# ipc-sim/IPC

Measured on NVIDIA H100. Metric: newton_iteration_ms_assembly_ccd, lower is better.
Workload: dtype f64

## Files before the change

ipc_b200/csrc/abi.h:

```cpp
#pragma once
#include "../../include/ipcgpu.h"
#include "common.cuh"
#include "context.h"
#include <cstddef>
#include <string>

#define CK(call)                                                                                  \
    do {                                                                                          \
        cudaError_t e_ = (call);                                                                  \
        if (e_ != cudaSuccess) {                                                                  \
            ctx->err = std::string(#call) + ": " + cudaGetErrorString(e_);                        \
            return IPCGPU_ERR_CUDA;                                                               \
        }                                                                                         \
    } while (0)
#define REQUIRE(cond, code, msg)                                                                  \
    do {                                                                                          \
        if (!(cond)) {                                                                            \
            ctx->err = (msg);                                                                     \
            return (code);                                                                        \
        }                                                                                         \
    } while (0)
#define ALLOC(buf, count) REQUIRE((buf).reserve(count), IPCGPU_ERR_CUDA, "cudaMalloc failed for " #buf)

static inline int nblk(long long n, int b) { return (int)((n + b - 1) / b); }

enum Chain { kSerial, kStepBound, kDerivative };

inline int join_deriv(ipcgpu_ctx* ctx)
{
    if (!ctx->deriv_open) return IPCGPU_OK;
    ctx->deriv_open = false;
    CK(cudaEventRecord(ctx->ev_deriv_done, ctx->deriv));
    CK(cudaStreamWaitEvent(ctx->stream, ctx->ev_deriv_done, 0));
    return IPCGPU_OK;
}

inline int enter(ipcgpu_ctx* ctx, Chain chain)
{
    CK(cudaSetDevice(ctx->device));
    if (chain == kStepBound) return IPCGPU_OK;
    if (chain == kSerial || ctx->nranks > 1 || ctx->profiling) return join_deriv(ctx);
    if (ctx->deriv_open) return IPCGPU_OK;
    CK(cudaEventRecord(ctx->ev_deriv_fork, ctx->stream));
    CK(cudaStreamWaitEvent(ctx->deriv, ctx->ev_deriv_fork, 0));
    ctx->deriv_open = true;
    return IPCGPU_OK;
}
#define ENTER(chain)                                                                              \
    do {                                                                                          \
        int re_ = enter(ctx, (chain));                                                            \
        if (re_) return re_;                                                                      \
    } while (0)

int join_copy_stream(ipcgpu_ctx* ctx);
int fetch_iter_state(ipcgpu_ctx* ctx);
int sync_pattern_mirror(ipcgpu_ctx* ctx);
int flag_status(ipcgpu_ctx* ctx, unsigned mask);
void set_local(ipcgpu_ctx* ctx, unsigned bits, bool local);
int energy_result(ipcgpu_ctx* ctx, int slot, double* E, bool fetch = false, unsigned check = 0);
int energy_tail(ipcgpu_ctx* ctx, int slot, const double* partials, int n_partials, double scale, cudaEvent_t pe, double* E, bool fetch = false,
    unsigned check = 0, const double* scale_dev = nullptr);

inline bool kappa_on_device(double kappa) { return kappa == IPCGPU_KAPPA_DEVICE; }
inline const double* kappa_ptr(ipcgpu_ctx* ctx, double kappa) { return kappa_on_device(kappa) ? &ctx->iter.p->kappa : nullptr; }
#define REQUIRE_KAPPA(kappa)                                                                                                        \
    REQUIRE(!kappa_on_device(kappa) || ctx->nranks == 1, IPCGPU_ERR_STATE, "the device-resident kappa (IPCGPU_KAPPA_DEVICE) runs on one rank")
int gradient_roundtrip_begin(ipcgpu_ctx* ctx, const double* g_in);
int gradient_roundtrip_end(ipcgpu_ctx* ctx, double* g_out);
int hessian_begin(ipcgpu_ctx* ctx, Chain chain, const double* a_inout);
int hessian_end(ipcgpu_ctx* ctx, double* a_inout, unsigned check);

int nccl_sum(ipcgpu_ctx* ctx, double* buf, size_t n, const char* what);
int nccl_sum(ipcgpu_ctx* ctx, int* buf, size_t n, const char* what);
int nccl_min_u64(ipcgpu_ctx* ctx, unsigned long long* word);
int nccl_all_gather(ipcgpu_ctx* ctx, const int4* send, int4* recv, size_t n, const char* what);
void nccl_comm_destroy(ipcgpu_ctx* ctx);

int build_maps(ipcgpu_ctx* ctx);
void owned_value_range(ipcgpu_ctx* ctx);
int ensure_offsets(ipcgpu_ctx* ctx);
int upload_dir(ipcgpu_ctx* ctx, const double* p);

int timestep_prepare(ipcgpu_ctx* ctx, ipcgpu::DynamicsArgs* p);

namespace ipcgpu {
struct SortedGrid;
}
int contact_alloc(ipcgpu_ctx* ctx);
int contact_constraint_set(ipcgpu_ctx* ctx, double dHat, int wantCand, int* nC, int* nPara, int* nCand);
int contact_sync_counts(ipcgpu_ctx* ctx);
void contact_pack_lists(ipcgpu_ctx* ctx);
void contact_unpack_lists(ipcgpu_ctx* ctx);
ipcgpu::SurfArgs surf_args(const ipcgpu_ctx* ctx);
ipcgpu::BarrierArgs barrier_args(ipcgpu_ctx* ctx, double dHat, double kappa, int projectDBC);
ipcgpu::HalfSpaceArgs halfspace_args(ipcgpu_ctx* ctx);
ipcgpu::SortedGrid edge_grid(const ipcgpu_ctx* ctx);
int boxes_and_grid(ipcgpu_ctx* ctx, double radius, bool with_vertex_boxes);

int ccd_alloc(ipcgpu_ctx* ctx);
int ccd_narrow(ipcgpu_ctx* ctx, const int2* cand, const int* n32, const unsigned long long* n64, unsigned long long cap, int share, double tol, const double* err_vf,
    const double* err_ee, int stage, const int* overflow);
int ccd_build_swept(ipcgpu_ctx* ctx, double h);
int ccd_full(ipcgpu_ctx* ctx, double tol, const double* err_vf, const double* err_ee);
int ccd_read_back(ipcgpu_ctx* ctx, double* alpha_out);

int decide(ipcgpu_ctx* ctx, int op, double a, int b, cudaGraphConditionalHandle h, bool* word, const double* aux = nullptr);
int cond_prepare(ipcgpu_ctx* ctx, const char* what);

template <typename Body>
int cond_node(ipcgpu_ctx* ctx, bool loop, int op, double a, int b, Body body)
{
    int rc;
    if (!ctx->capturing) {
        bool go = false;
        if ((rc = decide(ctx, op, a, b, 0, &go))) return rc;
        while (go) {
            if ((rc = body())) return rc;
            if (!loop) break;
            if ((rc = decide(ctx, op, a, b, 0, &go))) return rc;
        }
        return IPCGPU_OK;
    }
    REQUIRE(ctx->cond_depth < ipcgpu_ctx::kCondDepth, IPCGPU_ERR_STATE, "conditional nodes nested too deeply");
    cudaStreamCaptureStatus cs;
    cudaGraph_t g = nullptr;
    const cudaGraphNode_t* deps = nullptr;
    size_t nd = 0;
    CK(cudaStreamGetCaptureInfo(ctx->stream, &cs, nullptr, &g, &deps, &nd));
    cudaGraphConditionalHandle h = 0;
    const cudaError_t eh = cudaGraphConditionalHandleCreate(&h, g, 0, 0);
    if (eh != cudaSuccess) {
        cudaGetLastError();
        ctx->err = std::string("conditional graph nodes need CUDA 12.4 or newer in the driver: ") + cudaGetErrorString(eh);
        return IPCGPU_ERR_CUDA;
    }
    if ((rc = decide(ctx, op, a, b, h, nullptr))) return rc;
    CK(cudaStreamGetCaptureInfo(ctx->stream, &cs, nullptr, &g, &deps, &nd));
    cudaGraphNodeParams np = {};
    np.type = cudaGraphNodeTypeConditional;
    np.conditional.handle = h;
    np.conditional.type = loop ? cudaGraphCondTypeWhile : cudaGraphCondTypeIf;
    np.conditional.size = 1;
    cudaGraphNode_t node;
    CK(cudaGraphAddNode(&node, g, deps, nd, &np));
    cudaGraph_t bg = np.conditional.phGraph_out[0];
    ctx->capture_bodies.push_back(bg);
    cudaStream_t outer = ctx->stream, inner = ctx->cond_streams[ctx->cond_depth];
    CK(cudaStreamBeginCaptureToGraph(inner, bg, nullptr, nullptr, 0, cudaStreamCaptureModeThreadLocal));
    ctx->stream = inner;
    ++ctx->cond_depth;
    ctx->inputs_marked = false;
    rc = body();
    if (!rc && loop) rc = decide(ctx, op, a, b, h, nullptr);
    --ctx->cond_depth;
    ctx->stream = outer;
    cudaGraph_t captured = nullptr;
    const cudaError_t ee = cudaStreamEndCapture(inner, &captured);
    if (rc) return rc;
    CK(ee);
    CK(cudaStreamUpdateCaptureDependencies(outer, &node, 1, cudaStreamSetCaptureDependencies));
    ctx->mark_inputs();
    return IPCGPU_OK;
}

constexpr int kKrylovBurst = 25;
int solver_finish(ipcgpu_ctx* ctx);
template <typename Iteration>
int krylov_loops(ipcgpu_ctx* ctx, int max_iter, Iteration iteration)
{
    for (const int burst : { kKrylovBurst, max_iter % kKrylovBurst }) {
        if (burst == 0 || burst > max_iter) continue;
        int rc = cond_node(ctx, true, ipcgpu::kSolveBurst, 0.0, burst, [&]() {
            for (int k = 0; k < burst; ++k) iteration();
            CK(cudaGetLastError());
            return IPCGPU_OK;
        });
        if (rc) return rc;
    }
    return solver_finish(ctx);
}
int solver_full_pattern(ipcgpu_ctx* ctx);
int solver_forget_full_pattern(ipcgpu_ctx* ctx);
constexpr int kPcgSpmvBlocks = ipcgpu::kSMs * 8;
int solver_pcg(ipcgpu_ctx* ctx, const double* rhs_dev, double sign, double rel_tol, int max_iter, bool multilevel);
// ... 37 lines not shown
```

ipc_b200/csrc/ccd.cu:

```cuda
#include "broadphase.cuh"
#include "abi.h"
#include <cub/cub.cuh>

namespace ipcgpu {

__global__ void __launch_bounds__(256) k_ref_ranges(SurfArgs s, const double* __restrict__ dir, const IterState* __restrict__ st, int* __restrict__ vmin, int* __restrict__ vmax)
{
    const int i = blockIdx.x * blockDim.x + threadIdx.x;
    if (i >= s.nSV) return;
    const double alpha = st->alpha_grid, inv_h = st->ref_inv_h;
    const int v = s.SVI[i];
#pragma unroll
    for (int c = 0; c < 3; ++c) {
        const double x = s.V[(size_t)c * s.nV + v];
        const double xt = x + alpha * dir[3 * (size_t)v + c];
        const int a = (int)floor((x - st->ref_lo[c]) * inv_h), b = (int)floor((xt - st->ref_lo[c]) * inv_h);
        vmin[3 * (size_t)v + c] = min(a, b);
        vmax[3 * (size_t)v + c] = max(a, b);
    }
}

__global__ void __launch_bounds__(256) k_swept_bounds(SurfArgs s, const double* __restrict__ dir, const IterState* __restrict__ st, unsigned long long* __restrict__ bounds)
{
    __shared__ double sm[6][8];
    const double alpha = st->alpha_grid;
    double r[6] = { 1e300, 1e300, 1e300, -1e300, -1e300, -1e300 };
    for (int i = blockIdx.x * blockDim.x + threadIdx.x; i < max(s.nV, s.nSV); i += gridDim.x * blockDim.x) {
        if (i < s.nV) {
#pragma unroll
            for (int c = 0; c < 3; ++c) {
                const double x = s.V[(size_t)c * s.nV + i];
                r[c] = fmin(r[c], x);
                r[3 + c] = fmax(r[3 + c], x);
            }
        }
        if (i < s.nSV) {
            const int v = s.SVI[i];
#pragma unroll
            for (int c = 0; c < 3; ++c) {
                const double xt = s.V[(size_t)c * s.nV + v] + alpha * dir[3 * (size_t)v + c];
                r[c] = fmin(r[c], xt);
                r[3 + c] = fmax(r[3 + c], xt);
            }
        }
    }
#pragma unroll
    for (int q = 0; q < 6; ++q) {
        double x = r[q];
#pragma unroll
        for (int o = 16; o > 0; o >>= 1) {
            const double y = __shfl_xor_sync(0xffffffffu, x, o);
            x = q < 3 ? fmin(x, y) : fmax(x, y);
        }
        if ((threadIdx.x & 31) == 0) sm[q][threadIdx.x >> 5] = x;
    }
    __syncthreads();
    if (threadIdx.x < 6) {
        const int q = threadIdx.x;
        double x = sm[q][0];
        for (int w = 1; w < (int)(blockDim.x >> 5); ++w) x = q < 3 ? fmin(x, sm[q][w]) : fmax(x, sm[q][w]);
        if (q < 3) atomicMin(bounds + q, flip_ord(x));
        else atomicMax(bounds + q, flip_ord(x));
    }
}

__global__ void k_swept_alpha(IterState* st, const double* __restrict__ pSize_ptr, double h, unsigned long long* __restrict__ bounds)
{
    if (threadIdx.x != 0) return;
    const double pSize = *pSize_ptr;
    double alpha = ord_to_dbl(st->step_ord);
    const double span = alpha * pSize / h;
    if (span > 1) alpha /= span;
    st->step_ord = dbl_to_ord(alpha);
    st->alpha_grid = alpha;
    st->alpha_stage[2] = alpha;
    for (int c = 0; c < 3; ++c) { bounds[c] = ~0ull; bounds[3 + c] = 0ull; }
}
__global__ void k_refgrid_params(IterState* st, const unsigned long long* __restrict__ bounds, double h, SweptCells* __restrict__ sc)
{
    if (threadIdx.x != 0) return;
    sc->lmax = 0;
    sc->hmax[0] = sc->hmax[1] = sc->hmax[2] = 0;
    double lo[3], hi[3], rmax = 0.0;
    double inv_h = 1.0 / h;
    bool bad = false;
    for (int c = 0; c < 3; ++c) {
        lo[c] = unflip_ord(bounds[c]);
        hi[c] = unflip_ord(bounds[3 + c]);
        st->ref_lo[c] = lo[c];
        st->ref_count[c] = (int)ceil((hi[c] - lo[c]) * inv_h);
        rmax = fmax(rmax, hi[c] - lo[c]);
        if (st->ref_count[c] <= 0) bad = true;
    }
    if (bad) {
        inv_h = 1.0 / (rmax * 1.01);
        st->ref_count[0] = st->ref_count[1] = st->ref_count[2] = 1;
    }
    st->ref_inv_h = inv_h;
}

constexpr int kSweptExactK = 65534;

DEV bool ranges_overlap(const int* alo, const int* ahi, const int* blo, const int* bhi)
{
    return !(blo[0] > ahi[0] || bhi[0] < alo[0] || blo[1] > ahi[1] || bhi[1] < alo[1] || blo[2] > ahi[2] || bhi[2] < alo[2]);
}
DEV void prim_range(const int* __restrict__ vmin, const int* __restrict__ vmax, const int* vs, int n, int* lo, int* hi)
{
#pragma unroll
    for (int c = 0; c < 3; ++c) {
        lo[c] = vmin[3 * (size_t)vs[0] + c];
        hi[c] = vmax[3 * (size_t)vs[0] + c];
        for (int k = 1; k < n; ++k) {
            lo[c] = min(lo[c], vmin[3 * (size_t)vs[k] + c]);
            hi[c] = max(hi[c], vmax[3 * (size_t)vs[k] + c]);
        }
    }
}
DEV bool dbc_v(const SurfArgs& s, int v) { return s.dbc && s.dbc[v] != 0; }
DEV int cod_v(const SurfArgs& s, int v) { return s.vCoDim ? s.vCoDim[v] : 3; }

DEV int swept_prim(const SurfArgs& s, int i, int* vs, int& id)
{
    if (i < s.nSF) {
        id = i;
        vs[0] = s.SF[i]; vs[1] = s.SF[(size_t)s.nSF + i]; vs[2] = s.SF[(size_t)2 * s.nSF + i];
        return 3;
    }
    i -= s.nSF;
    if (i < s.nSE) {
        id = i;
        vs[0] = s.SE[2 * i]; vs[1] = s.SE[2 * i + 1];
        return 2;
    }
    id = i - s.nSE;
    vs[0] = s.SVI[id];
    return 1;
}

__global__ void __launch_bounds__(256) k_swept_extent(SurfArgs s, const int* __restrict__ vmin, const int* __restrict__ vmax, SweptCells* __restrict__ sc)
{
    __shared__ int sm[4][8];
    int r[4] = { 0, 0, 0, 0 };
    for (int i = blockIdx.x * blockDim.x + threadIdx.x; i < s.nSF + s.nSE + s.nSV; i += gridDim.x * blockDim.x) {
        int vs[3], id, lo[3], hi[3];
        const int nv = swept_prim(s, i, vs, id);
        prim_range(vmin, vmax, vs, nv, lo, hi);
        for (int c = 0; c < 3; ++c) {
            r[0] = max(r[0], hi[c] - lo[c] + 1);
            r[1 + c] = max(r[1 + c], hi[c]);
        }
    }
    for (int q = 0; q < 4; ++q) {
        r[q] = __reduce_max_sync(0xffffffffu, r[q]);
        if ((threadIdx.x & 31) == 0) sm[q][threadIdx.x >> 5] = r[q];
    }
    __syncthreads();
    if (threadIdx.x < 4) {
        int x = 0;
        for (int w = 0; w < (int)(blockDim.x >> 5); ++w) x = max(x, sm[threadIdx.x][w]);
        atomicMax(threadIdx.x == 0 ? &sc->lmax : &sc->hmax[threadIdx.x - 1], x);
    }
}
__global__ void k_swept_cells(SweptCells* sc)
{
    if (threadIdx.x != 0) return;
    auto fits = [&](long long K) {
        unsigned long long n = 1;
        for (int c = 0; c < 3; ++c) n *= (unsigned long long)(sc->hmax[c] / K + 1);
        return n <= (unsigned long long)kGridCells;
    };
    long long lo = max(2, sc->lmax - 1);
    if (!fits(lo)) {
        long long hi = (long long)max(sc->hmax[0], max(sc->hmax[1], sc->hmax[2])) + 1;
        while (hi - lo > 1) {
            const long long mid = (lo + hi) / 2;
            if (fits(mid)) hi = mid;
            else lo = mid;
        }
        lo = hi;
    }
    const int K = (int)min(lo, 0x7fffffffll);
    sc->K = K;
    for (int c = 0; c < 3; ++c) sc->n[c] = sc->hmax[c] / K + 1;
}
DEV unsigned swept_key(const SweptCells& g, int type, int x, int y, int z) { return ((unsigned)type << kGridCellsLog2) | (unsigned)((z * g.n[1] + y) * g.n[0] + x); }

__global__ void __launch_bounds__(256) k_swept_count(SurfArgs s, const int* __restrict__ vmin, const int* __restrict__ vmax, const SweptCells* __restrict__ sc,
    int* __restrict__ cnt)
{
    const int i = blockIdx.x * blockDim.x + threadIdx.x;
    if (i >= s.nSF + s.nSE + s.nSV) return;
    const SweptCells g = *sc;
    int vs[3], id, lo[3], hi[3];
    const int nv = swept_prim(s, i, vs, id);
    prim_range(vmin, vmax, vs, nv, lo, hi);
    for (int z = lo[2] / g.K; z <= hi[2] / g.K; ++z)
        for (int y = lo[1] / g.K; y <= hi[1] / g.K; ++y)
            for (int x = lo[0] / g.K; x <= hi[0] / g.K; ++x) atomicAdd(cnt + swept_key(g, 3 - nv, x, y, z), 1);
}
__global__ void __launch_bounds__(256) k_swept_scatter(SurfArgs s, const int* __restrict__ vmin, const int* __restrict__ vmax, const SweptCells* __restrict__ sc,
    int* __restrict__ cnt, const int* __restrict__ off, unsigned* __restrict__ keys, uint4* __restrict__ ent)
{
    const int i = blockIdx.x * blockDim.x + threadIdx.x;
    if (i >= s.nSF + s.nSE + s.nSV) return;
    const SweptCells g = *sc;
    int vs[3], id, lo[3], hi[3];
    const int nv = swept_prim(s, i, vs, id);
    prim_range(vmin, vmax, vs, nv, lo, hi);
    auto rel = [&](int v, int c) { return (unsigned)min(max((long long)v - ((long long)g.K * c - 1), 0ll), 65535ll); };
    for (int z = lo[2] / g.K; z <= hi[2] / g.K; ++z)
        for (int y = lo[1] / g.K; y <= hi[1] / g.K; ++y)
            for (int x = lo[0] / g.K; x <= hi[0] / g.K; ++x) {
                const unsigned key = swept_key(g, 3 - nv, x, y, z);
                const int pos = off[key] + atomicSub(cnt + key, 1) - 1;
                keys[pos] = key;
                ent[pos] = make_uint4(rel(lo[0], x) | (rel(lo[1], y) << 16), rel(lo[2], z) | (rel(hi[0], x) << 16), rel(hi[1], y) | (rel(hi[2], z) << 16), (unsigned)id);
            }
}

DEV bool swept_hit(const uint4& a, const uint4& b)
{
    const unsigned M01 = __vmaxu2(a.x, b.x), m01 = __vminu2(__funnelshift_r(a.y, a.z, 16), __funnelshift_r(b.y, b.z, 16));
    const unsigned M2 = max(a.y & 0xffffu, b.y & 0xffffu), m2 = min(a.z >> 16, b.z >> 16);
    return __vcmpleu2(M01, m01) == 0xffffffffu && (M01 & 0xffffu) != 0u && (M01 >> 16) != 0u && M2 != 0u && M2 <= m2;
}

struct CandOut {
    int2* cand;
    unsigned long long* n;
    unsigned long long cap;
    int* overflow;
};
DEV void push_cand(const CandOut& o, int2 c)
{
    const unsigned m = __activemask();
    const int lane = threadIdx.x & 31, leader = __ffs(m) - 1;
    unsigned long long base = 0;
    if (lane == leader) base = atomicAdd(o.n, (unsigned long long)__popc(m));
    base = __shfl_sync(m, base, leader);
    const unsigned long long i = base + __popc(m & ((1u << lane) - 1u));
    if (i < o.cap) o.cand[i] = c;
    else atomicExch(o.overflow, 1);
}

struct SweptArgs {
    SurfArgs s;
    const double* dir;
    const IterState* st;
    const int *vmin, *vmax;
    const SweptCells* sc;
    const unsigned* keys;
    const uint4* ent;
    const int* off;
    int lo, hi;
    CandOut out;
};

DEV void pt_candidate(const SweptArgs& a, bool wide, int svI, int sfI)
{
    const SurfArgs& s = a.s;
    const int vI = s.SVI[svI];
    const int tv[3] = { s.SF[sfI], s.SF[(size_t)s.nSF + sfI], s.SF[(size_t)2 * s.nSF + sfI] };
    if (wide) {
        int lo[3], hi[3];
        prim_range(a.vmin, a.vmax, tv, 3, lo, hi);
        if (!ranges_overlap(a.vmin + 3 * (size_t)vI, a.vmax + 3 * (size_t)vI, lo, hi)) return;
    }
    const bool oP = obstacle_vertex(s, vI), oT = obstacle_vertex(s, tv[0]);
    if (oP && oT) return;
    if (!oP && !oT && ((cod_v(s, vI) < 3 && cod_v(s, tv[0]) < 3) || (dbc_v(s, vI) && dbc_v(s, tv[0]) && dbc_v(s, tv[1]) && dbc_v(s, tv[2])))) return;
    push_cand(a.out, make_int2(-svI - 1, sfI));
}
DEV void ee_candidate(const SweptArgs& a, bool wide, int eI, int eJ)
{
    const SurfArgs& s = a.s;
    if (eI < a.lo || eI >= a.hi) return;
    const int v[4] = { s.SE[2 * eI], s.SE[2 * eI + 1], s.SE[2 * eJ], s.SE[2 * eJ + 1] };
    if (wide) {
        int qlo[3], qhi[3], lo[3], hi[3];
        prim_range(a.vmin, a.vmax, v, 2, qlo, qhi);
        prim_range(a.vmin, a.vmax, v + 2, 2, lo, hi);
        if (!ranges_overlap(qlo, qhi, lo, hi)) return;
    }
    {
        const double alpha = a.st->alpha_grid;
        double blo[2][3], bhi[2][3];
#pragma unroll
        for (int e = 0; e < 2; ++e)
#pragma unroll
            for (int c = 0; c < 3; ++c) {
                blo[e][c] = 1e300;
                bhi[e][c] = -1e300;
#pragma unroll
                for (int k = 0; k < 2; ++k) {
                    const int w = v[2 * e + k];
                    const double x = __ldg(s.V + (size_t)c * s.nV + w), xt = x + alpha * __ldg(a.dir + 3 * (size_t)w + c);
                    blo[e][c] = fmin(fmin(blo[e][c], x), xt);
                    bhi[e][c] = fmax(fmax(bhi[e][c], x), xt);
                }
            }
// ... 1083 lines not shown
                            ms_in = 0.0; tolerance_in = a.tol; t_max = max_t0; iter = 0; is_impacting = false; best = nullptr;
                            restart = true;
                        }
                        else {
                            if (attempt == 1 && hit) toi *= 0.8;
                            finished = true;
                        }
                    }
                }
                if (restart) {
                    width_tolerances(vf, P, tolerance_in, tol);
#pragma unroll
                    for (int d = 0; d < 3; ++d) inv_tol[d] = 1.0 / tol[d];
                    bfs1_init(bf, bufA, bufB, tolerance_in, best);
                    out_tol = tolerance_in;
                }
                if (finished) {
                    if (hit == 1) atomicMin(min_ord, dbl_to_ord(toi));
                    busy = false;
                }
            }
        }
    }
}

__global__ void __launch_bounds__(128, 2) k_ti_stage2(NarrowArgs a, const unsigned* __restrict__ survivors, const unsigned* __restrict__ nSurvPtr, unsigned* __restrict__ work,
    DBox* __restrict__ scratch, int cap, unsigned long long* __restrict__ min_ord, int* __restrict__ warn)
{
    __shared__ DBox sLevels[kStage2WarpsPerCtaDev][2][kSmemLevel];
    __shared__ TiPair sPair[kStage2WarpsPerCtaDev];
    const int lane = threadIdx.x & 31;
    const int warp_global = (blockIdx.x * blockDim.x + threadIdx.x) >> 5;
    DBox* sA = sLevels[threadIdx.x >> 5][0];
    DBox* sB = sLevels[threadIdx.x >> 5][1];
    DBox* bufA = scratch + (size_t)warp_global * 2 * cap;
    DBox* bufB = bufA + cap;
    const unsigned nSurv = *nSurvPtr;
    unsigned long long boxes = 0;
    for (;;) {
        unsigned w = 0;
        if (lane == 0) w = atomicAdd(work, 1u);
        w = __shfl_sync(0xffffffffu, w, 0);
        if (w >= nSurv) {
            if (lane == 0 && boxes) atomicAdd(reinterpret_cast<unsigned long long*>(warn + 7), boxes);
            break;
        }
        bool vf;
        {
            int v[4];
            TiPair Pl;
            load_pair(a.s, a.dir, a.cand[survivors[w]], vf, v, Pl);
            if (lane == 0) sPair[threadIdx.x >> 5] = Pl;
            __syncwarp();
        }
        const TiPair& P = sPair[threadIdx.x >> 5];
        double toi;
        const long long t0 = clock64();
        const int hit = pair_ccd(vf, P, a, bufA, bufB, cap, lane, toi, warn, boxes, sA, sB);
        if (hit && lane == 0) atomicMin(min_ord, dbl_to_ord(toi));
        if (lane == 0) {
            const unsigned dt = (unsigned)((clock64() - t0) >> 6);
            atomicMax(reinterpret_cast<unsigned*>(warn + 3), dt);
            atomicAdd(reinterpret_cast<unsigned*>(warn + 4), dt);
        }
        __syncwarp();
    }
}

__global__ void k_ccd_init(IterState* st, const int* __restrict__ n32, const unsigned long long* __restrict__ n64, unsigned long long cap, int rank, int nranks, int share,
    double seed, unsigned* nSurv, unsigned* work, int* flags)
{
    if (threadIdx.x != 0) return;
    const double alpha = ord_to_dbl(st->step_ord);
    st->max_t = alpha;
    st->ccd_ord = (seed >= 0.0 && seed < alpha) ? dbl_to_ord(seed) : st->step_ord;
    unsigned long long n = n32 ? (unsigned long long)max(*n32, 0) : *n64;
    if (n > cap) n = cap;
    st->cand_range[0] = share ? n * rank / nranks : 0ull;
    st->cand_range[1] = share ? n * (rank + 1) / nranks : n;
    *nSurv = 0;
    *work = 0;
    for (int q = 0; q < 12; ++q) flags[q] = 0;
}
__global__ void k_ccd_finish(IterState* st, const unsigned* __restrict__ nSurv, const int* __restrict__ flags, const int* __restrict__ overflow, int is_full)
{
    if (threadIdx.x != 0) return;
    if (flags[0]) {
        st->ccd_ord = 0ull;
        st->flags[FLAG_ZERO_CCD_DISTANCE] = 1;
    }
    if (overflow && *overflow) st->flags[FLAG_CCD_CAPACITY] = 1;
    st->flags[FLAG_TI_WARNINGS] += flags[1];
    st->ccd_stats[0] = *nSurv;
    st->ccd_stats[1] = (unsigned long long)flags[1];
    st->ccd_stats[2] = (unsigned)flags[2];
    st->ccd_stats[3] = (unsigned long long)(unsigned)flags[4] << 6;
    st->ccd_stats[4] = (unsigned long long)(unsigned)flags[5] << 6;
    st->ccd_stats[5] = *reinterpret_cast<const unsigned long long*>(flags + 6);
    st->ccd_stats[6] = *reinterpret_cast<const unsigned long long*>(flags + 8);
    st->ccd_stats[7] = st->cand_range[1] - st->cand_range[0];
    if (is_full) st->n_full_cand = st->ccd_stats[7];
}
__global__ void k_ccd_commit(IterState* st, int stage)
{
    if (threadIdx.x != 0) return;
    st->step_ord = st->ccd_ord;
    st->alpha_stage[stage] = ord_to_dbl(st->ccd_ord);
}

}

using namespace ipcgpu;


constexpr int kStage2WarpsPerCta = 4;
constexpr int kStage2Ctas = kSMs * 2;
constexpr int kLevelCap = 4096;

int ccd_alloc(ipcgpu_ctx* ctx)
{
    CcdWork& w = ctx->ccd;
    const size_t warps = (size_t)kStage2Ctas * kStage2WarpsPerCta;
    const size_t nEnt = (size_t)8 * std::max(ctx->nSF + ctx->nSE + ctx->nSV, 1);
    size_t scan_bytes = 0;
    cub::DeviceScan::ExclusiveSum(nullptr, scan_bytes, (int*)nullptr, (int*)nullptr, (int)(3 * kGridCells + 1));
    if (!w.arena_lock.p) {
        if (!w.arena_lock.reserve(1) || cudaMemsetAsync(w.arena_lock.p, 0, sizeof(int), ctx->stream) != cudaSuccess) {
            ctx->err = "CCD workspace allocation failed";
            return IPCGPU_ERR_CUDA;
        }
    }
    bool ok = w.arena.reserve((size_t)2 * kArenaLevel * sizeof(DBox)) && w.vmin.reserve((size_t)3 * ctx->nV) && w.vmax.reserve((size_t)3 * ctx->nV) && w.cand.reserve(ctx->ccd_capacity) && w.surv.reserve(ctx->ccd_capacity) && w.surv2.reserve(ctx->ccd_capacity)
        && w.scratch.reserve(warps * 2 * kLevelCap * sizeof(DBox)) && w.counters.reserve(16) && w.ncand.reserve(2) && w.bounds.reserve(8) && w.cells.reserve(1)
        && w.sw_keys.reserve(nEnt) && w.sw_ent.reserve(nEnt) && w.sw_cnt.reserve((size_t)3 * kGridCells + 1) && w.sw_off.reserve((size_t)3 * kGridCells + 1)
        && w.sw_tmp.reserve(scan_bytes + 256);
    if (!ok) {
        ctx->err = "CCD workspace allocation failed";
        return IPCGPU_ERR_CUDA;
    }
    return 0;
}

int ccd_narrow(ipcgpu_ctx* ctx, const int2* cand, const int* n32, const unsigned long long* n64, unsigned long long cap, int share, double tol, const double* err_vf,
    const double* err_ee, int stage, const int* overflow)
{
    CcdWork& w = ctx->ccd;
    cudaStream_t st = ctx->stream;
    NarrowArgs a;
    a.s = surf_args(ctx);
    a.dir = ctx->dir.p;
    a.cand = cand;
    for (int c = 0; c < 3; ++c) { a.err_vf[c] = err_vf[c]; a.err_ee[c] = err_ee[c]; }
    a.tol = tol;
    a.max_itr = 1000000;
    a.st = ctx->iter.p;
    a.arena = reinterpret_cast<DBox*>(w.arena.p);
    a.arena_lock = w.arena_lock.p;
    IterState* ist = ctx->iter.p;
    unsigned* nSurv = reinterpret_cast<unsigned*>(w.counters.p);
    unsigned* work = nSurv + 1;
    int* flags = w.counters.p + 2;
    cudaEvent_t pe = ctx->prof_begin(IPCGPU_STAGE_CCD_NARROW);
    k_ccd_init<<<1, 32, 0, st>>>(ist, n32, n64, cap, ctx->rank, ctx->nranks, share, ctx->debug_prune_seed, nSurv, work, flags);
    {
        cudaEvent_t pe1 = ctx->prof_begin(IPCGPU_STAGE_CCD_ROOT_FILTER);
        k_ti_stage1<<<kSMs * 16, 128, 0, st>>>(a, w.surv.p, nSurv, flags);
        ctx->prof_end(pe1);
        unsigned* nDefA = reinterpret_cast<unsigned*>(flags + 2);
        unsigned* refill_work = reinterpret_cast<unsigned*>(flags + 3);
        constexpr long long kThreadBudget = 96;
        const long long budget = ctx->debug_ti_budget >= 0 ? ctx->debug_ti_budget : kThreadBudget;
        constexpr int bytes = 2 * 128 * (kThreadLevel * (int)sizeof(DBox) + 8);
        static bool attr = false;
        if (!attr) { CK(cudaFuncSetAttribute(k_ti_stage15_refill, cudaFuncAttributeMaxDynamicSharedMemorySize, bytes)); attr = true; }
        k_ti_stage15_refill<<<kSMs * 2, 128, bytes, st>>>(a, w.surv.p, nSurv, refill_work, w.surv2.p, nDefA, budget, &ist->ccd_ord, flags + 1);
        k_ti_stage2<<<kStage2Ctas, 32 * kStage2WarpsPerCta, 0, st>>>(a, w.surv2.p, nDefA, work, reinterpret_cast<DBox*>(w.scratch.p), kLevelCap, &ist->ccd_ord, flags + 1);
    }
    k_ccd_finish<<<1, 32, 0, st>>>(ist, nSurv, flags, overflow, stage == 3);
    ctx->prof_end(pe);
    ctx->launches += 5;
    CK(cudaGetLastError());
    int rc = nccl_min_u64(ctx, &ist->ccd_ord);
    if (rc) return rc;
    k_ccd_commit<<<1, 32, 0, st>>>(ist, stage);
    ++ctx->launches;
    return 0;
}

int ccd_read_back(ipcgpu_ctx* ctx, double* alpha_out)
{
    int rc = fetch_iter_state(ctx);
    if (rc) return rc;
    CcdWork& w = ctx->ccd;
    const IterState& h = *ctx->h_iter;
    w.last_survivors = (unsigned)h.ccd_stats[0];
    w.last_warnings = (int)h.ccd_stats[1];
    w.last_deferred = h.ccd_stats[2];
    w.last_longest_cycles = h.ccd_stats[3];
    w.last_total_cycles = h.ccd_stats[4];
    w.last_boxes_thread = h.ccd_stats[5];
    w.last_boxes_warp = h.ccd_stats[6];
    w.last_candidates = h.ccd_stats[7];
    if (alpha_out) std::memcpy(alpha_out, &h.step_ord, sizeof(double));
    return 0;
}

int ccd_build_swept(ipcgpu_ctx* ctx, double h)
{
    CcdWork& w = ctx->ccd;
    cudaStream_t st = ctx->stream;
    const SurfArgs s = surf_args(ctx);
    IterState* ist = ctx->iter.p;
    if (!ctx->dir_valid) {
        ctx->err = "no search direction: pass p (or call ipcgpu_set_search_dir first)";
        return IPCGPU_ERR_STATE;
    }
    cudaEvent_t pe = ctx->prof_begin(IPCGPU_STAGE_CCD_BROAD);
    k_swept_alpha<<<1, 32, 0, st>>>(ist, ctx->pSize_dev.p, h, w.bounds.p);
    k_swept_bounds<<<std::min(nblk(std::max(s.nV, s.nSV), 256), kSMs * 4), 256, 0, st>>>(s, ctx->dir.p, ist, w.bounds.p);
    k_refgrid_params<<<1, 32, 0, st>>>(ist, w.bounds.p, h, w.cells.p);
    ctx->launches += 3;
    const int nPrim = s.nSF + s.nSE + s.nSV;
    if (s.nSV > 0) {
        k_ref_ranges<<<nblk(s.nSV, 256), 256, 0, st>>>(s, ctx->dir.p, ist, w.vmin.p, w.vmax.p);
        k_swept_extent<<<std::min(nblk(nPrim, 256), kSMs * 4), 256, 0, st>>>(s, w.vmin.p, w.vmax.p, w.cells.p);
        k_swept_cells<<<1, 32, 0, st>>>(w.cells.p);
        const size_t nTab = (size_t)3 * kGridCells + 1;
        zero_words(w.sw_cnt.p, nTab, st);
        k_swept_count<<<nblk(nPrim, 256), 256, 0, st>>>(s, w.vmin.p, w.vmax.p, w.cells.p, w.sw_cnt.p);
        size_t bytes = w.sw_tmp.n;
        CK(cub::DeviceScan::ExclusiveSum(w.sw_tmp.p, bytes, w.sw_cnt.p, w.sw_off.p, (int)nTab, st));
        k_swept_scatter<<<nblk(nPrim, 256), 256, 0, st>>>(s, w.vmin.p, w.vmax.p, w.cells.p, w.sw_cnt.p, w.sw_off.p, w.sw_keys.p, w.sw_ent.p);
        ctx->launches += 7;
    }
    ctx->prof_end(pe);
    CK(cudaGetLastError());
    w.swept_ready = true;
    return 0;
}

int ccd_full(ipcgpu_ctx* ctx, double tol, const double* err_vf, const double* err_ee)
{
    CcdWork& w = ctx->ccd;
    cudaStream_t st = ctx->stream;
    const SurfArgs s = surf_args(ctx);
    cudaEvent_t pe = ctx->prof_begin(IPCGPU_STAGE_CCD_BROAD);
    CK(cudaMemsetAsync(w.ncand.p, 0, 2 * sizeof(unsigned long long), st));
    CK(cudaMemsetAsync(w.counters.p + 14, 0, sizeof(int), st));
    SweptArgs a{ s, ctx->dir.p, ctx->iter.p, w.vmin.p, w.vmax.p, w.cells.p, w.sw_keys.p, w.sw_ent.p, w.sw_off.p, 0, 0,
        CandOut{ w.cand.p, w.ncand.p, (unsigned long long)ctx->ccd_capacity, w.counters.p + 14 } };
    if (s.nSF > 0 && s.nSV > 0) {
        a.lo = (int)((long long)s.nSV * ctx->rank / ctx->nranks);
        a.hi = (int)((long long)s.nSV * (ctx->rank + 1) / ctx->nranks);
        k_swept_pairs_pt<<<kSMs * 8, 32 * kSweptWarps, 0, st>>>(a);
        ++ctx->launches;
    }
    if (s.nSE > 1) {
        a.lo = (int)((long long)s.nSE * ctx->rank / ctx->nranks);
        a.hi = (int)((long long)s.nSE * (ctx->rank + 1) / ctx->nranks);
        k_swept_pairs_ee<<<kSMs * 8, 32 * kSweptWarps, 0, st>>>(a);
        ++ctx->launches;
    }
    ctx->prof_end(pe);
    return ccd_narrow(ctx, w.cand.p, nullptr, w.ncand.p, (unsigned long long)ctx->ccd_capacity, 0, tol, err_vf, err_ee, 3, w.counters.p + 14);
}
```

Measured before the change: 2.522.

## Fuse swept-grid setup kernels via last-CTA tickets and warp-aggregate cell atomics

Folds the single-thread alpha, refgrid-params and cell-sizing kernels into the preceding reduction kernels, using a last-CTA ticket so that one block finishes the serial tail. Per-iteration memsets are dropped: the buffers are zeroed once at allocation and then restored by the consumers (the scatter decrements counts back to zero, and finish clears the candidate counters). Count and scatter walk cells per warp and use match_any so that threads with the same cell key share one atomic. Pair-kernel grid size now comes from an occupancy query instead of a fixed 8 blocks per SM. The aim is fewer graph nodes and less serial-launch latency, in exchange for relying on buffers returning to a zeroed state after each iteration.

```diff
diff --git a/ipc_b200/csrc/abi.h b/ipc_b200/csrc/abi.h
--- a/ipc_b200/csrc/abi.h
+++ b/ipc_b200/csrc/abi.h
@@ -98,8 +98,8 @@
 int boxes_and_grid(ipcgpu_ctx* ctx, double radius, bool with_vertex_boxes);
 
 int ccd_alloc(ipcgpu_ctx* ctx);
-int ccd_narrow(ipcgpu_ctx* ctx, const int2* cand, const int* n32, const unsigned long long* n64, unsigned long long cap, int share, double tol, const double* err_vf,
-    const double* err_ee, int stage, const int* overflow);
+int ccd_narrow(ipcgpu_ctx* ctx, const int2* cand, const int* n32, unsigned long long* n64, unsigned long long cap, int share, double tol, const double* err_vf,
+    const double* err_ee, int stage, int* overflow);
 int ccd_build_swept(ipcgpu_ctx* ctx, double h);
 int ccd_full(ipcgpu_ctx* ctx, double tol, const double* err_vf, const double* err_ee);
 int ccd_read_back(ipcgpu_ctx* ctx, double* alpha_out);
diff --git a/ipc_b200/csrc/ccd.cu b/ipc_b200/csrc/ccd.cu
--- a/ipc_b200/csrc/ccd.cu
+++ b/ipc_b200/csrc/ccd.cu
@@ -20,10 +20,54 @@
     }
 }
 
-__global__ void __launch_bounds__(256) k_swept_bounds(SurfArgs s, const double* __restrict__ dir, const IterState* __restrict__ st, unsigned long long* __restrict__ bounds)
+DEV double swept_alpha(const IterState* st, const double* __restrict__ pSize_ptr, double h)
+{
+    const double pSize = *pSize_ptr;
+    double alpha = ord_to_dbl(st->step_ord);
+    const double span = alpha * pSize / h;
+    if (span > 1) alpha /= span;
+    return alpha;
+}
+DEV void refgrid_params(IterState* st, const unsigned long long* bounds, double h, SweptCells* __restrict__ sc)
+{
+    sc->lmax = 0;
+    sc->hmax[0] = sc->hmax[1] = sc->hmax[2] = 0;
+    double lo[3], hi[3], rmax = 0.0;
+    double inv_h = 1.0 / h;
+    bool bad = false;
+    for (int c = 0; c < 3; ++c) {
+        lo[c] = unflip_ord(__ldcg(bounds + c));
+        hi[c] = unflip_ord(__ldcg(bounds + 3 + c));
+        st->ref_lo[c] = lo[c];
+        st->ref_count[c] = (int)ceil((hi[c] - lo[c]) * inv_h);
+        rmax = fmax(rmax, hi[c] - lo[c]);
+        if (st->ref_count[c] <= 0) bad = true;
+    }
+    if (bad) {
+        inv_h = 1.0 / (rmax * 1.01);
+        st->ref_count[0] = st->ref_count[1] = st->ref_count[2] = 1;
+    }
+    st->ref_inv_h = inv_h;
+}
+
+DEV bool last_cta(unsigned long long* ticket)
+{
+    __shared__ bool last;
+    __threadfence();
+    __syncthreads();
+    if (threadIdx.x == 0) {
+        last = atomicAdd(ticket, 1ull) == (unsigned long long)(gridDim.x - 1);
+        if (last) *ticket = 0ull;
+    }
+    __syncthreads();
+    return last;
+}
+
+__global__ void __launch_bounds__(256) k_swept_bounds(SurfArgs s, const double* __restrict__ dir, IterState* st, const double* __restrict__ pSize_ptr, double h,
+    unsigned long long* __restrict__ bounds, SweptCells* __restrict__ sc)
 {
     __shared__ double sm[6][8];
-    const double alpha = st->alpha_grid;
+    const double alpha = swept_alpha(st, pSize_ptr, h);
     double r[6] = { 1e300, 1e300, 1e300, -1e300, -1e300, -1e300 };
     for (int i = blockIdx.x * blockDim.x + threadIdx.x; i < max(s.nV, s.nSV); i += gridDim.x * blockDim.x) {
         if (i < s.nV) {
@@ -62,41 +106,12 @@
         if (q < 3) atomicMin(bounds + q, flip_ord(x));
         else atomicMax(bounds + q, flip_ord(x));
     }
-}
-
-__global__ void k_swept_alpha(IterState* st, const double* __restrict__ pSize_ptr, double h, unsigned long long* __restrict__ bounds)
-{
-    if (threadIdx.x != 0) return;
-    const double pSize = *pSize_ptr;
-    double alpha = ord_to_dbl(st->step_ord);
-    const double span = alpha * pSize / h;
-    if (span > 1) alpha /= span;
+    if (!last_cta(bounds + 6) || threadIdx.x != 0) return;
     st->step_ord = dbl_to_ord(alpha);
     st->alpha_grid = alpha;
     st->alpha_stage[2] = alpha;
+    refgrid_params(st, bounds, h, sc);
     for (int c = 0; c < 3; ++c) { bounds[c] = ~0ull; bounds[3 + c] = 0ull; }
-}
-__global__ void k_refgrid_params(IterState* st, const unsigned long long* __restrict__ bounds, double h, SweptCells* __restrict__ sc)
-{
-    if (threadIdx.x != 0) return;
-    sc->lmax = 0;
-    sc->hmax[0] = sc->hmax[1] = sc->hmax[2] = 0;
-    double lo[3], hi[3], rmax = 0.0;
-    double inv_h = 1.0 / h;
-    bool bad = false;
-    for (int c = 0; c < 3; ++c) {
-        lo[c] = unflip_ord(bounds[c]);
-        hi[c] = unflip_ord(bounds[3 + c]);
-        st->ref_lo[c] = lo[c];
-        st->ref_count[c] = (int)ceil((hi[c] - lo[c]) * inv_h);
-        rmax = fmax(rmax, hi[c] - lo[c]);
-        if (st->ref_count[c] <= 0) bad = true;
-    }
-    if (bad) {
-        inv_h = 1.0 / (rmax * 1.01);
-        st->ref_count[0] = st->ref_count[1] = st->ref_count[2] = 1;
-    }
-    st->ref_inv_h = inv_h;
 }
 
 constexpr int kSweptExactK = 65534;
@@ -138,7 +153,31 @@
     return 1;
 }
 
-__global__ void __launch_bounds__(256) k_swept_extent(SurfArgs s, const int* __restrict__ vmin, const int* __restrict__ vmax, SweptCells* __restrict__ sc)
+DEV void swept_cells(SweptCells* sc)
+{
+    const int lmax = __ldcg(&sc->lmax), hmax[3] = { __ldcg(&sc->hmax[0]), __ldcg(&sc->hmax[1]), __ldcg(&sc->hmax[2]) };
+    auto fits = [&](long long K) {
+        unsigned long long n = 1;
+        for (int c = 0; c < 3; ++c) n *= (unsigned long long)(hmax[c] / K + 1);
+        return n <= (unsigned long long)kGridCells;
+    };
+    long long lo = max(2, lmax - 1);
+    if (!fits(lo)) {
+        long long hi = (long long)max(hmax[0], max(hmax[1], hmax[2])) + 1;
+        while (hi - lo > 1) {
+            const long long mid = (lo + hi) / 2;
+            if (fits(mid)) hi = mid;
+            else lo = mid;
+        }
+        lo = hi;
+    }
+    const int K = (int)min(lo, 0x7fffffffll);
+    sc->K = K;
+    for (int c = 0; c < 3; ++c) sc->n[c] = hmax[c] / K + 1;
+}
+
+__global__ void __launch_bounds__(256) k_swept_extent(SurfArgs s, const int* __restrict__ vmin, const int* __restrict__ vmax, SweptCells* __restrict__ sc,
+    unsigned long long* __restrict__ ticket)
 {
     __shared__ int sm[4][8];
     int r[4] = { 0, 0, 0, 0 };
@@ -161,62 +200,69 @@
         for (int w = 0; w < (int)(blockDim.x >> 5); ++w) x = max(x, sm[threadIdx.x][w]);
         atomicMax(threadIdx.x == 0 ? &sc->lmax : &sc->hmax[threadIdx.x - 1], x);
     }
-}
-__global__ void k_swept_cells(SweptCells* sc)
-{
-    if (threadIdx.x != 0) return;
-    auto fits = [&](long long K) {
-        unsigned long long n = 1;
-        for (int c = 0; c < 3; ++c) n *= (unsigned long long)(sc->hmax[c] / K + 1);
-        return n <= (unsigned long long)kGridCells;
-    };
-    long long lo = max(2, sc->lmax - 1);
-    if (!fits(lo)) {
-        long long hi = (long long)max(sc->hmax[0], max(sc->hmax[1], sc->hmax[2])) + 1;
-        while (hi - lo > 1) {
-            const long long mid = (lo + hi) / 2;
-            if (fits(mid)) hi = mid;
-            else lo = mid;
-        }
-        lo = hi;
-    }
-    const int K = (int)min(lo, 0x7fffffffll);
-    sc->K = K;
-    for (int c = 0; c < 3; ++c) sc->n[c] = sc->hmax[c] / K + 1;
+    if (last_cta(ticket) && threadIdx.x == 0) swept_cells(sc);
 }
 DEV unsigned swept_key(const SweptCells& g, int type, int x, int y, int z) { return ((unsigned)type << kGridCellsLog2) | (unsigned)((z * g.n[1] + y) * g.n[0] + x); }
+
+template <typename F> DEV void for_each_cell_warp(const SweptCells& g, const int* lo, const int* hi, bool valid, F f)
+{
+    int c0[3], nc[3];
+#pragma unroll
+    for (int c = 0; c < 3; ++c) {
+        c0[c] = lo[c] / g.K;
+        nc[c] = hi[c] / g.K - c0[c] + 1;
+    }
+    const int n = valid ? nc[0] * nc[1] * nc[2] : 0;
+    const int nmax = (int)__reduce_max_sync(0xffffffffu, (unsigned)n);
+    for (int k = 0; k < nmax; ++k) {
+        const bool on = k < n;
+        const unsigned act = __ballot_sync(0xffffffffu, on);
+        if (on) f(act, c0[0] + k % nc[0], c0[1] + (k / nc[0]) % nc[1], c0[2] + k / (nc[0] * nc[1]));
+    }
+}
 
 __global__ void __launch_bounds__(256) k_swept_count(SurfArgs s, const int* __restrict__ vmin, const int* __restrict__ vmax, const SweptCells* __restrict__ sc,
     int* __restrict__ cnt)
 {
     const int i = blockIdx.x * blockDim.x + threadIdx.x;
-    if (i >= s.nSF + s.nSE + s.nSV) return;
+    const bool valid = i < s.nSF + s.nSE + s.nSV;
+    const int lane = threadIdx.x & 31;
     const SweptCells g = *sc;
-    int vs[3], id, lo[3], hi[3];
-    const int nv = swept_prim(s, i, vs, id);
-    prim_range(vmin, vmax, vs, nv, lo, hi);
-    for (int z = lo[2] / g.K; z <= hi[2] / g.K; ++z)
-        for (int y = lo[1] / g.K; y <= hi[1] / g.K; ++y)
-            for (int x = lo[0] / g.K; x <= hi[0] / g.K; ++x) atomicAdd(cnt + swept_key(g, 3 - nv, x, y, z), 1);
+    int vs[3], id, lo[3] = { 0, 0, 0 }, hi[3] = { 0, 0, 0 }, nv = 0;
+    if (valid) {
+        nv = swept_prim(s, i, vs, id);
+        prim_range(vmin, vmax, vs, nv, lo, hi);
+    }
+    for_each_cell_warp(g, lo, hi, valid, [&](unsigned act, int x, int y, int z) {
+        const unsigned key = swept_key(g, 3 - nv, x, y, z);
+        const unsigned peers = __match_any_sync(act, key);
+        if (lane == __ffs(peers) - 1) atomicAdd(cnt + key, __popc(peers));
+    });
 }
 __global__ void __launch_bounds__(256) k_swept_scatter(SurfArgs s, const int* __restrict__ vmin, const int* __restrict__ vmax, const SweptCells* __restrict__ sc,
     int* __restrict__ cnt, const int* __restrict__ off, unsigned* __restrict__ keys, uint4* __restrict__ ent)
 {
     const int i = blockIdx.x * blockDim.x + threadIdx.x;
-    if (i >= s.nSF + s.nSE + s.nSV) return;
+    const bool valid = i < s.nSF + s.nSE + s.nSV;
+    const int lane = threadIdx.x & 31;
     const SweptCells g = *sc;
-    int vs[3], id, lo[3], hi[3];
-    const int nv = swept_prim(s, i, vs, id);
-    prim_range(vmin, vmax, vs, nv, lo, hi);
+    int vs[3], id = 0, lo[3] = { 0, 0, 0 }, hi[3] = { 0, 0, 0 }, nv = 0;
+    if (valid) {
+        nv = swept_prim(s, i, vs, id);
+        prim_range(vmin, vmax, vs, nv, lo, hi);
+    }
     auto rel = [&](int v, int c) { return (unsigned)min(max((long long)v - ((long long)g.K * c - 1), 0ll), 65535ll); };
-    for (int z = lo[2] / g.K; z <= hi[2] / g.K; ++z)
-        for (int y = lo[1] / g.K; y <= hi[1] / g.K; ++y)
-            for (int x = lo[0] / g.K; x <= hi[0] / g.K; ++x) {
-                const unsigned key = swept_key(g, 3 - nv, x, y, z);
-                const int pos = off[key] + atomicSub(cnt + key, 1) - 1;
-                keys[pos] = key;
-                ent[pos] = make_uint4(rel(lo[0], x) | (rel(lo[1], y) << 16), rel(lo[2], z) | (rel(hi[0], x) << 16), rel(hi[1], y) | (rel(hi[2], z) << 16), (unsigned)id);
-            }
+    for_each_cell_warp(g, lo, hi, valid, [&](unsigned act, int x, int y, int z) {
+        const unsigned key = swept_key(g, 3 - nv, x, y, z);
+        const unsigned peers = __match_any_sync(act, key);
+        const int leader = __ffs(peers) - 1;
+        int top = 0;
+        if (lane == leader) top = atomicSub(cnt + key, __popc(peers));
+        top = __shfl_sync(act, top, leader);
+        const int pos = off[key] + top - 1 - __popc(peers & ((1u << lane) - 1u));
+        keys[pos] = key;
+        ent[pos] = make_uint4(rel(lo[0], x) | (rel(lo[1], y) << 16), rel(lo[2], z) | (rel(hi[0], x) << 16), rel(hi[1], y) | (rel(hi[2], z) << 16), (unsigned)id);
+    });
 }
 
 DEV bool swept_hit(const uint4& a, const uint4& b)
@@ -1466,7 +1512,8 @@
     *work = 0;
     for (int q = 0; q < 12; ++q) flags[q] = 0;
 }
-__global__ void k_ccd_finish(IterState* st, const unsigned* __restrict__ nSurv, const int* __restrict__ flags, const int* __restrict__ overflow, int is_full)
+__global__ void k_ccd_finish(IterState* st, const unsigned* __restrict__ nSurv, const int* __restrict__ flags, int* __restrict__ overflow,
+    unsigned long long* __restrict__ n64, int is_full)
 {
     if (threadIdx.x != 0) return;
     if (flags[0]) {
@@ -1474,6 +1521,10 @@
         st->flags[FLAG_ZERO_CCD_DISTANCE] = 1;
     }
     if (overflow && *overflow) st->flags[FLAG_CCD_CAPACITY] = 1;
+    if (is_full) {
+        *overflow = 0;
+        *n64 = 0ull;
+    }
     st->flags[FLAG_TI_WARNINGS] += flags[1];
     st->ccd_stats[0] = *nSurv;
     st->ccd_stats[1] = (unsigned long long)flags[1];
@@ -1518,6 +1569,11 @@
         && w.scratch.reserve(warps * 2 * kLevelCap * sizeof(DBox)) && w.counters.reserve(16) && w.ncand.reserve(2) && w.bounds.reserve(8) && w.cells.reserve(1)
         && w.sw_keys.reserve(nEnt) && w.sw_ent.reserve(nEnt) && w.sw_cnt.reserve((size_t)3 * kGridCells + 1) && w.sw_off.reserve((size_t)3 * kGridCells + 1)
         && w.sw_tmp.reserve(scan_bytes + 256);
+    ok = ok && cudaMemsetAsync(w.bounds.p, 0xff, 3 * sizeof(unsigned long long), ctx->stream) == cudaSuccess
+        && cudaMemsetAsync(w.bounds.p + 3, 0, 5 * sizeof(unsigned long long), ctx->stream) == cudaSuccess
+        && cudaMemsetAsync(w.sw_cnt.p, 0, w.sw_cnt.n * sizeof(int), ctx->stream) == cudaSuccess
+        && cudaMemsetAsync(w.ncand.p, 0, w.ncand.n * sizeof(unsigned long long), ctx->stream) == cudaSuccess
+        && cudaMemsetAsync(w.counters.p, 0, w.counters.n * sizeof(int), ctx->stream) == cudaSuccess;
     if (!ok) {
         ctx->err = "CCD workspace allocation failed";
         return IPCGPU_ERR_CUDA;
@@ -1525,8 +1581,8 @@
     return 0;
 }
 
-int ccd_narrow(ipcgpu_ctx* ctx, const int2* cand, const int* n32, const unsigned long long* n64, unsigned long long cap, int share, double tol, const double* err_vf,
-    const double* err_ee, int stage, const int* overflow)
+int ccd_narrow(ipcgpu_ctx* ctx, const int2* cand, const int* n32, unsigned long long* n64, unsigned long long cap, int share, double tol, const double* err_vf,
+    const double* err_ee, int stage, int* overflow)
 {
     CcdWork& w = ctx->ccd;
     cudaStream_t st = ctx->stream;
@@ -1560,7 +1616,7 @@
         k_ti_stage15_refill<<<kSMs * 2, 128, bytes, st>>>(a, w.surv.p, nSurv, refill_work, w.surv2.p, nDefA, budget, &ist->ccd_ord, flags + 1);
         k_ti_stage2<<<kStage2Ctas, 32 * kStage2WarpsPerCta, 0, st>>>(a, w.surv2.p, nDefA, work, reinterpret_cast<DBox*>(w.scratch.p), kLevelCap, &ist->ccd_ord, flags + 1);
     }
-    k_ccd_finish<<<1, 32, 0, st>>>(ist, nSurv, flags, overflow, stage == 3);
+    k_ccd_finish<<<1, 32, 0, st>>>(ist, nSurv, flags, overflow, n64, stage == 3);
     ctx->prof_end(pe);
     ctx->launches += 5;
     CK(cudaGetLastError());
@@ -1600,22 +1656,18 @@
         return IPCGPU_ERR_STATE;
     }
     cudaEvent_t pe = ctx->prof_begin(IPCGPU_STAGE_CCD_BROAD);
-    k_swept_alpha<<<1, 32, 0, st>>>(ist, ctx->pSize_dev.p, h, w.bounds.p);
-    k_swept_bounds<<<std::min(nblk(std::max(s.nV, s.nSV), 256), kSMs * 4), 256, 0, st>>>(s, ctx->dir.p, ist, w.bounds.p);
-    k_refgrid_params<<<1, 32, 0, st>>>(ist, w.bounds.p, h, w.cells.p);
-    ctx->launches += 3;
+    k_swept_bounds<<<std::min(nblk(std::max(s.nV, s.nSV), 256), kSMs * 4), 256, 0, st>>>(s, ctx->dir.p, ist, ctx->pSize_dev.p, h, w.bounds.p, w.cells.p);
+    ++ctx->launches;
     const int nPrim = s.nSF + s.nSE + s.nSV;
     if (s.nSV > 0) {
         k_ref_ranges<<<nblk(s.nSV, 256), 256, 0, st>>>(s, ctx->dir.p, ist, w.vmin.p, w.vmax.p);
-        k_swept_extent<<<std::min(nblk(nPrim, 256), kSMs * 4), 256, 0, st>>>(s, w.vmin.p, w.vmax.p, w.cells.p);
-        k_swept_cells<<<1, 32, 0, st>>>(w.cells.p);
+        k_swept_extent<<<std::min(nblk(nPrim, 256), kSMs * 4), 256, 0, st>>>(s, w.vmin.p, w.vmax.p, w.cells.p, w.bounds.p + 7);
         const size_t nTab = (size_t)3 * kGridCells + 1;
-        zero_words(w.sw_cnt.p, nTab, st);
         k_swept_count<<<nblk(nPrim, 256), 256, 0, st>>>(s, w.vmin.p, w.vmax.p, w.cells.p, w.sw_cnt.p);
         size_t bytes = w.sw_tmp.n;
         CK(cub::DeviceScan::ExclusiveSum(w.sw_tmp.p, bytes, w.sw_cnt.p, w.sw_off.p, (int)nTab, st));
         k_swept_scatter<<<nblk(nPrim, 256), 256, 0, st>>>(s, w.vmin.p, w.vmax.p, w.cells.p, w.sw_cnt.p, w.sw_off.p, w.sw_keys.p, w.sw_ent.p);
-        ctx->launches += 7;
+        ctx->launches += 5;
     }
     ctx->prof_end(pe);
     CK(cudaGetLastError());
@@ -1629,20 +1681,25 @@
     cudaStream_t st = ctx->stream;
     const SurfArgs s = surf_args(ctx);
     cudaEvent_t pe = ctx->prof_begin(IPCGPU_STAGE_CCD_BROAD);
-    CK(cudaMemsetAsync(w.ncand.p, 0, 2 * sizeof(unsigned long long), st));
-    CK(cudaMemsetAsync(w.counters.p + 14, 0, sizeof(int), st));
     SweptArgs a{ s, ctx->dir.p, ctx->iter.p, w.vmin.p, w.vmax.p, w.cells.p, w.sw_keys.p, w.sw_ent.p, w.sw_off.p, 0, 0,
         CandOut{ w.cand.p, w.ncand.p, (unsigned long long)ctx->ccd_capacity, w.counters.p + 14 } };
+    static int waves[2] = { 0, 0 };
+    if (!waves[0]) {
+        CK(cudaOccupancyMaxActiveBlocksPerMultiprocessor(&waves[0], k_swept_pairs_pt, 32 * kSweptWarps, 0));
+        CK(cudaOccupancyMaxActiveBlocksPerMultiprocessor(&waves[1], k_swept_pairs_ee, 32 * kSweptWarps, 0));
+        waves[0] = std::max(waves[0], 1);
+        waves[1] = std::max(waves[1], 1);
+    }
     if (s.nSF > 0 && s.nSV > 0) {
         a.lo = (int)((long long)s.nSV * ctx->rank / ctx->nranks);
         a.hi = (int)((long long)s.nSV * (ctx->rank + 1) / ctx->nranks);
-        k_swept_pairs_pt<<<kSMs * 8, 32 * kSweptWarps, 0, st>>>(a);
+        k_swept_pairs_pt<<<kSMs * waves[0], 32 * kSweptWarps, 0, st>>>(a);
         ++ctx->launches;
     }
     if (s.nSE > 1) {
         a.lo = (int)((long long)s.nSE * ctx->rank / ctx->nranks);
         a.hi = (int)((long long)s.nSE * (ctx->rank + 1) / ctx->nranks);
-        k_swept_pairs_ee<<<kSMs * 8, 32 * kSweptWarps, 0, st>>>(a);
+        k_swept_pairs_ee<<<kSMs * waves[1], 32 * kSweptWarps, 0, st>>>(a);
         ++ctx->launches;
     }
     ctx->prof_end(pe);
diff --git a/profiles/swept_chain_timing.py b/profiles/swept_chain_timing.py
--- /dev/null
+++ b/profiles/swept_chain_timing.py
@@ -0,0 +1,125 @@
+import argparse
+import json
+import os
+import sys
+import tempfile
+
+import numpy as np
+
+ROOT = os.path.dirname(os.path.dirname(os.path.abspath(__file__)))
+sys.path.insert(0, ROOT)
+sys.path.insert(0, os.path.join(ROOT, "profiles"))
+
+import bench
+from device_pattern_timing import Args, gpu_info
+from ipc_b200 import lib as L
+
+DERIV = ("elastic", "assemble", "barrier", "gather", "diag_mass", "inertia", "reduce_sum", "para_gradient")
+
+
+def short(name):
+    n = name.split("(")[0].replace("void ", "").replace("ipcgpu::", "")
+    if "cub::" in name:
+        n = "cub::" + n.split("::")[-1].split("<")[0]
+    return n
+
+
+def main():
+    ap = argparse.ArgumentParser()
+    ap.add_argument("--reps", type=int, default=20)
+    args = ap.parse_args()
+    import torch
+    from torch.profiler import ProfilerActivity, profile
+
+    m, info = bench.build_scene(Args())
+    dHat, h = info["dHat"], m.avgEdgeLen / 3.0
+    ctx = L.Context(0)
+    ctx.set_mesh(m.V_rest_soa, m.T_soa, m.restTriInv, m.vol, m.mu, m.lam, m.mass, m.dbc, m.energy)
+    ctx.set_surface(m.SVI, m.SFEdges, m.SF_soa, m.vCoDim)
+    ctx.set_state(m.V_soa)
+    evf, eee = L.Context.ti_error(m.V_soa, m.nV, None)
+    mm, pa, pe, _ = ctx.constraint_set(dHat, 1)
+    ia, ja = m.csr_pattern(1, extra_pairs=bench.contact_pattern_pairs(m, mm, pa, pe))
+    ctx.set_csr(ia, ja, 1)
+    ctx.set_contact_partition(1)
+    ctx.set_canonical_order(0)
+    ctx.set_search_dir(info["p"])
+
+    def enqueue_iteration():
+        ctx.constraint_set(dHat, 1, fetch=False, sizes=False)
+        ctx.barrier_energy(dHat, bench.KAPPA, want=False)
+        ctx.elastic_energy_grad_hess(bench.DT2, 1, 1, 1, None, None)
+        ctx.barrier_gradient(dHat, bench.KAPPA, None)
+        ctx.barrier_hessian(dHat, bench.KAPPA, 1, None)
+        ctx.allreduce_grad_hess(1, 0)
+        ctx.step_bound_set(1.0)
+        ctx.inversion_step(None, 0.2, None)
+        ctx.ccd_partial(None, bench.TI_TOL, evf, eee, None)
+        ctx.hash_build_swept(None, None, h)
+        ctx.ccd_full(bench.TI_TOL, evf, eee, None)
+
+    for _ in range(3):
+        enqueue_iteration()
+        ctx.fetch_iteration()
+    ctx.capture_begin()
+    enqueue_iteration()
+    graph = ctx.capture_end()
+    for _ in range(5):
+        ctx.graph_launch(graph)
+        ctx.fetch_iteration()
+    ctx.timer_start()
+    for _ in range(args.reps):
+        ctx.graph_launch(graph)
+        ctx.fetch_iteration()
+    iter_ms = ctx.timer_stop() / args.reps
+    with profile(activities=[ProfilerActivity.CUDA]) as prof:
+        for _ in range(args.reps):
+            ctx.graph_launch(graph)
+            ctx.fetch_iteration()
+        torch.cuda.synchronize()
+    with tempfile.TemporaryDirectory() as d:
+        path = os.path.join(d, "trace.json")
+        prof.export_chrome_trace(path)
+        ev = json.load(open(path))["traceEvents"]
+    gpu = sorted(({"name": short(e["name"]), "ts": float(e["ts"]), "end": float(e["ts"]) + float(e.get("dur", 0)), "memset": e.get("cat") == "gpu_memset", "tid": e.get("tid")}
+                  for e in ev if e.get("cat") in ("kernel", "gpu_memset")), key=lambda e: e["ts"])
+    commits = [e for e in gpu if e["name"] == "k_ccd_commit"]
+    streams = {e["tid"] for e in gpu if e["name"].startswith("k_swept")}
+    spans, busy, nodes, waits, per_node = [], [], None, [], {}
+    for c in commits[0::2]:
+        t0 = c["end"]
+        t1 = next((e["ts"] for e in gpu if e["ts"] > t0 and e["name"] == "k_ti_stage15_refill"), None)
+        if t1 is None:
+            continue
+        chain = [e for e in gpu if t0 <= e["ts"] < t1 and (e["tid"] in streams or e["memset"]) and not any(k in e["name"] for k in DERIV)]
+        cover, hi = 0.0, t0
+        for e in chain:
+            lo_, hi_ = max(e["ts"], hi), min(e["end"], t1)
+            if hi_ > lo_:
+                cover += hi_ - lo_
+            hi = max(hi, min(e["end"], t1))
+        spans.append(t1 - t0)
+        busy.append(cover)
+        prev = t0
+        w = []
+        for e in chain:
+            per_node.setdefault(e["name"], []).append(e["end"] - e["ts"])
+            if e["memset"]:
+                w.append(round(e["ts"] - prev, 2))
+            prev = max(prev, e["end"])
+        waits.append(w)
+        if nodes is None:
+            nodes = [e["name"] for e in chain]
+    med = lambda x: round(float(np.median(x)), 2)
+    out = {"gpu": gpu_info(), "scene": f"C5, {m.nT} tets", "reps": args.reps, "iteration_ms": round(iter_ms, 4),
+           "gpu_nodes_per_iteration": len(gpu) / args.reps, "iterations_traced": len(spans),
+           "span_us": med(spans), "busy_us": med(busy), "gap_us": med(np.subtract(spans, busy)),
+           "memset_wait_us": [med([w[k] for w in waits if len(w) > k]) for k in range(max((len(w) for w in waits), default=0))],
+           "n_nodes": len(nodes or []), "nodes": nodes,
+           "node_us": {k: round(sum(v) / len(spans), 2) for k, v in per_node.items()}, "streams": sorted(map(str, streams))}
+    print(json.dumps(out))
+    ctx.close()
+
+
+if __name__ == "__main__":
+    main()
```

Result: faster. 2.491 (median of 6 runs) (-1.2%).
